# agwi-lab/renderformer

Hardware: AMD Instinct MI355X
Metric: rendered frames/sec at 512×512, renderformer-v1.1-swin-large, 1/2/4/8 MI355X (higher is better)
Workload: dtype fp16+bf16

## Files before the change

### renderformer_amd/csrc/gemm.hip

```cpp
#include <algorithm>
#include <type_traits>
#include <cmath>
#include <math.h>
#include <stdio.h>
#include <stdlib.h>
#include <string.h>

#include "common.h"
#include "env.h"

namespace {

constexpr int BK = 32;
constexpr int P_F16 = 2;

enum Epi { E_BF16 = RF_EPI_BF16, E_F32 = RF_EPI_F32, E_ADD = RF_EPI_ADD_F32, E_SWIGLU = RF_EPI_SWIGLU, E_CONV = 16,
           E_ROPE = 17 };

template <int BM_, int BN_, int WGM_, int WGN_, int STAGES_, int KH_ = 1>
struct Tile {
    static constexpr int BM = BM_, BN = BN_, WGM = WGM_, WGN = WGN_, STAGES = STAGES_, KH = KH_;
    static constexpr int NWAVE = WGM * WGN, THREADS = NWAVE * 64;
    static constexpr int MW = BM / WGM, NWD = BN / WGN, TI = MW / 16, TJ = NWD / 16;
    static constexpr int APIECES = BM / 16;
    static constexpr bool ASHARE = APIECES < NWAVE;
    static constexpr int PA = ASHARE ? 1 : BM / 16 / NWAVE, PB = BN / 16 / NWAVE;
    static constexpr int A_BYTES = BM * BK * 2, B_BYTES = BN * BK * 2;
    static_assert(PA >= 1 && PB >= 1 && (ASHARE || PA * NWAVE * 16 == BM || BM == 288) && PB * NWAVE * 16 == BN,
                  "tile/wave mismatch");
    static_assert(TI >= 1 && TJ >= 2 && TJ % 2 == 0, "wave tile too small");
};

struct EngineArgs {
    const bf16_t* a;
    const bf16_t* a_lo;
    int64_t lda;
    const bf16_t* w;
    const bf16_t* w_lo;
    int64_t ldw;
    int m, n, k;
    int hi, wi, cin_pad, ho, wo, kw, stride, pad;
    uint64_t cin_m, kw_m;
    const bf16_t* zero;
// ... 12 lines not shown
    float elu_alpha;
    float* sk_part;
    int* sk_flag;
    int sk_epoch;
    int group_m;
    const int* gate;
    int halo_lg;
    int* err;
    int spin;
    uint64_t* stamps;
    const uint8_t* sa;
    const uint8_t* sw;
    int ld_sa, ld_sw;
    int persist;
    int l2pf;
    int out_f16;
    int* range;
    bf16_t* xg;
    int64_t ldxg;
    const float* norm_g;
    float* ss_out;
    int xg_f16;
    const float* rs_part;
    float rs_n, rs_eps;
    float* seg_ss;
    int seg_w, seg_n;
    const float* rope_pos;
    int64_t rope_ld;
    int rope_div;
    const float* rope_freqs;
// ... 2 lines not shown
    float rope_qscale;
};

constexpr int PN_SLOTS = RF_PRENORM_SLOTS;


RF_DEV uint32_t pack16(const EngineArgs& p, float lo, float hi) {
    return p.out_f16 ? pack_f16x2(lo, hi) : pack_bf16x2(lo, hi);
}

RF_DEV float unpack16(const EngineArgs& p, uint32_t h) {
    return p.out_f16 ? f16_bits_to_f32((uint16_t)h) : __uint_as_float(h << 16);
}

RF_DEV bool gated_off(const EngineArgs& p) { return p.gate && *p.gate == 0; }

RF_DEV int udiv_m(int x, uint64_t m) { return (int)(((uint64_t)(uint32_t)x * m) >> 32); }
inline uint64_t udiv_magic(int d) { return (1ull << 32) / (uint64_t)d + 1; }


RF_DEV void tile_coords(int tile, int tiles_m, int tiles_n, int group_m, int& tm, int& tn) {
    const int per_group = group_m * tiles_n;
    const int g = tile / per_group, r = tile - g * per_group;
    const int first = g * group_m;
    const int gm = min(tiles_m - first, group_m);
    tm = first + r % gm;
    tn = r / gm;
}

RF_DEV int lds_off(int row, int ch) { return row * 64 + ((ch ^ ((row >> 1) & 3)) << 4); }
// ... 86 lines not shown
    for (int pc = 0; pc < PA; ++pc) {
        int m = m0 + arow[pc];
        const bool ok = m < p.m;
        m = ok ? m : p.m - 1;
        g_img[pc] = g_iy[pc] = g_ix[pc] = 0;
        if constexpr (GATHER) {
            const int ox = m % p.wo, t = m / p.wo;
            g_img[pc] = ok ? t / p.ho : -1;
            g_iy[pc] = (t % p.ho) * p.stride - p.pad;
            g_ix[pc] = ox * p.stride - p.pad;
        }
        a_row[pc] = p.a + (int64_t)m * p.lda;
        a_row_lo[pc] = NTERM == 3 ? p.a_lo + (int64_t)m * p.lda : nullptr;
    }

    auto issue = [&](int kt, int buf) {
#pragma unroll
      for (int h = 0; h < KH; ++h) {
        char* st = smem + buf * STAGE_BYTES + h * HALF_BYTES;
        const int k0 = (kt * KH + h) * BK;
        int cb = k0, ky = 0, kx = 0;
        if constexpr (GATHER) {
            const int tap = udiv_m(k0, p.cin_m);
            cb = k0 - tap * p.cin_pad;
            ky = udiv_m(tap, p.kw_m);
            kx = tap - ky * p.kw;
        }
#pragma unroll
        for (int pc = 0; pc < PA; ++pc) {
            if (!stage_a) break;
            const int piece = wave * PA + pc;
            const int kofs = alc[pc] * 8;
            const bf16_t* sa;
            const bf16_t* sa_lo = nullptr;
            if constexpr (GATHER) {
// ... 587 lines not shown
            case 2: return (j >> 5) * 64 + (j & 31);
            default: return (j >> 5) * 64 + 32 + (j & 31);
        }
    } else {
        switch (r) {
            case 0: return j;
            case 1: return (j >> 5) * 64 + (j & 31);
            default: return (j >> 5) * 64 + 32 + (j & 31);
        }
    }
}
template <int ROWS>
RF_DEV int img(int row, int kh, int ch) { return kh * (ROWS * 64) + row * 64 + ((ch ^ ((row >> 1) & 3)) << 4); }
}

template <int BM, int NTERM, bool GATHER, bool INITC = false>
RF_DEV void phased_mainloop(const EngineArgs& p, char* smem, int m0, int n0, int kbeg, int kend,
                            f32x4 (&acc)[BM / 32][4], bool pre = false) {
    using namespace ph;
    using G = Cfg<BM>;
    constexpr int NREG = G::NREG, NA = G::NA, NX = G::NX, MI = G::MI;
    static_assert(NTERM == 1 || NTERM == P_F16, "phased loop: single-term operands");
    static_assert(!(GATHER && NX), "gathered A: no RAX region");
    constexpr int FA = G::FA, FA1 = G::FA1;
    const int lane = threadIdx.x & 63;
    const int wave = threadIdx.x >> 6;
    const int wr = wave >> 2, wc = wave & 3;
    const int nk = kend - kbeg;
    const bool has_a = BM >= 128 || __builtin_amdgcn_readfirstlane(wave) < BM / 16;
    const bool has_x = NX && (__builtin_amdgcn_readfirstlane(wave) & 3) == 0;

// ... 12 lines not shown
        const int m = m0 + trow[r];
        am[r] = m < p.m ? m : p.m - 1;
        src[r] = p.a + (int64_t)am[r] * p.lda;
        gi[r] = gy[r] = gx[r] = 0;
        if constexpr (GATHER) {
            const int ox = am[r] % p.wo, t = am[r] / p.wo;
            gi[r] = m < p.m ? t / p.ho : -1;
            gy[r] = (t % p.ho) * p.stride - p.pad;
            gx[r] = ox * p.stride - p.pad;
        }
    }
#pragma unroll
    for (int r = NA; r < NREG; ++r) src[r] = p.w + (int64_t)(n0 + trow[r]) * p.ldw;
    const int lch = lane & 3;

    auto issue = [&](int kt, int r) {
        const bool is_a = r < NA || r >= NREG;
        if (is_a && !has_a) return;
        if (r >= NREG && !has_x) return;
        char* base = smem + (kt & 1) * G::TILE + (is_a ? 0 : G::A_IMG);
#pragma unroll
        for (int kh = 0; kh < 2; ++kh) {
            const int row = trow[r];
            const int ch = lch ^ ((row >> 1) & 3);
            const int k0 = (kbeg + kt) * BK2 + kh * 32;
            const bf16_t* g = src[r] + k0 + ch * 8;
            if constexpr (GATHER) {
                if (r < NA) {
                    const int tap = udiv_m(k0, p.cin_m), cb = k0 - tap * p.cin_pad;
                    const int ky = udiv_m(tap, p.kw_m), kx = tap - ky * p.kw;
                    const int iy = gy[r] + ky, ix = gx[r] + kx;
                    const bool ok = gi[r] >= 0 && iy >= 0 && iy < p.hi && ix >= 0 && ix < p.wi;
                    g = ok ? p.a + (((int64_t)gi[r] * p.hi + iy) * p.wi + ix) * p.cin_pad + cb + ch * 8 : p.zero;
                }
            }
            char* dst = base + kh * (is_a ? BM * 64 : 256 * 64) + grow[r] * 64;
            __builtin_amdgcn_global_load_lds(GLB_PTR(void, g), LDS_PTR(void, dst), 16, 0, 0);
        }
    };

// ... 123 lines not shown
                issue(t + 2, 0);
                issue(t + 2, 1);
                if (has_a) wait_vm<4>();
                else wait_vm<2>();
            } else {
                wait_vm<0>();
            }
            sync_in();
            mma(0, 1, fb1);
            sync_out();
        }
    }
    if (!late) __builtin_amdgcn_s_barrier();
}

template <int BM, int NTERM, bool INITC>
RF_DEV void phased3_mainloop(const EngineArgs& p, char* smem, int m0, int n0, int kbeg, int kend,
                             f32x4 (&acc)[BM / 32][4], char* touch_lds = nullptr) {
    using namespace ph;
    using G = Cfg<BM>;
    static_assert(BM <= 128, "three-buffer loop: short tiles");
    constexpr int NREG = 3, FA = G::FA;
    const int lane = threadIdx.x & 63;
    const int wave = threadIdx.x >> 6;
    const int wr = wave >> 2, wc = wave & 3;
    const int nk = kend - kbeg;
    const bool has_a = BM >= 128 || __builtin_amdgcn_readfirstlane(wave) < BM / 16;
    const int jrow = 16 * wave + (lane >> 2);
    int trow[NREG], grow[NREG];
    const bf16_t* src[NREG];
#pragma unroll
    for (int r = 0; r < NREG; ++r) {
        trow[r] = region_row<BM>(r, jrow);
        grow[r] = region_row<BM>(r, 16 * wave);
    }
    {
        const int m = m0 + trow[0];
        src[0] = p.a + (int64_t)(m < p.m ? m : p.m - 1) * p.lda;
    }
#pragma unroll
    for (int r = 1; r < NREG; ++r) src[r] = p.w + (int64_t)(n0 + trow[r]) * p.ldw;
    const int lch = lane & 3;
    auto issue_tile = [&](int kt) {
        char* buf = smem + (kt % 3) * G::TILE;
#pragma unroll
        for (int r = 0; r < NREG; ++r) {
            const bool is_a = r == 0;
            if (is_a && !has_a) continue;
            char* base = buf + (is_a ? 0 : G::A_IMG);
#pragma unroll
            for (int kh = 0; kh < 2; ++kh) {
                const int row = trow[r];
                const int ch = lch ^ ((row >> 1) & 3);
                const int k0 = (kbeg + kt) * BK2 + kh * 32;
                char* dst = base + kh * (is_a ? BM * 64 : 256 * 64) + grow[r] * 64;
                __builtin_amdgcn_global_load_lds(GLB_PTR(void, src[r] + k0 + ch * 8), LDS_PTR(void, dst), 16, 0, 0);
            }
        }
    };
    const int l2pf = touch_lds ? p.l2pf : 0;
    const bf16_t* tsrc;
    {
        const int t = threadIdx.x;
        tsrc = t < BM ? p.a + (int64_t)min(m0 + t, p.m - 1) * p.lda
                      : p.w + (int64_t)(n0 + (t - BM) % 256) * p.ldw;
    }
    auto touch = [&](int kt) {
        const int kk = min(kt + l2pf, nk - 1);
        __builtin_amdgcn_global_load_lds(GLB_PTR(void, tsrc + (kbeg + kk) * BK2), LDS_PTR(void, touch_lds), 4, 0, 0);
    };
    if (INITC && kbeg == 0) {
        load_c_acc<BM / 32, 4>(p, m0 + wr * (BM / 2), n0 + wc * 64, acc);
    } else {
#pragma unroll
        for (int i = 0; i < BM / 32; ++i)
#pragma unroll
            for (int j = 0; j < 4; ++j) acc[i][j] = f32x4{0.f, 0.f, 0.f, 0.f};
    }
    const int frow = lane & 15, fch = lane >> 4;
    bf16x8 fa[FA][2], fb0[2][2], fb1[2][2];
    auto read_a = [&](const char* buf) {
#pragma unroll
        for (int i = 0; i < FA; ++i)
#pragma unroll
            for (int s = 0; s < 2; ++s)
                fa[i][s] = *reinterpret_cast<const bf16x8*>(buf + img<BM>(wr * (BM / 2) + i * 16 + frow, s, fch));
    };
    auto read_b = [&](const char* buf, int ni, bf16x8 (&fb)[2][2]) {
#pragma unroll
        for (int j = 0; j < 2; ++j)
#pragma unroll
            for (int s = 0; s < 2; ++s)
                fb[j][s] = *reinterpret_cast<const bf16x8*>(buf + G::A_IMG + img<256>(wc * 64 + ni * 32 + j * 16 + frow, s, fch));
    };
    auto mma = [&](int ni, const bf16x8 (&fb)[2][2]) {
        __builtin_amdgcn_s_setprio(1);
#pragma unroll
        for (int s = 0; s < 2; ++s)
#pragma unroll
            for (int i = 0; i < FA; ++i)
#pragma unroll
                for (int j = 0; j < 2; ++j) {
                    f32x4& c = acc[i][ni * 2 + j];
                    if constexpr (NTERM == P_F16)
                        c = __builtin_amdgcn_mfma_f32_16x16x32_f16(__builtin_bit_cast(f16x8, fb[j][s]),
                                                                   __builtin_bit_cast(f16x8, fa[i][s]), c, 0, 0, 0);
                    else
                        c = __builtin_amdgcn_mfma_f32_16x16x32_bf16(fb[j][s], fa[i][s], c, 0, 0, 0);
// ... 49 lines not shown
                else wait_vm<6>();
            } else {
                if (has_a) wait_vm<6>();
                else wait_vm<4>();
            }
        } else {
            wait_vm<0>();
        }
        sync_in();
        mma(1, fb1);
        sync_out();
    }
    if (!late) __builtin_amdgcn_s_barrier();
}

template <int BM, int EPI, int NTERM = 1>
__global__ __launch_bounds__(512, 1) void phased3_kernel(EngineArgs p) {
    using TE = Tile<BM, 256, 2, 4, 4>;
#ifdef RF_STUDY
    __shared__ __attribute__((aligned(16))) char smem[3 * ph::Cfg<BM>::TILE + PN_AREA<TE, EPI> + 256];
#else
    __shared__ __attribute__((aligned(16))) char smem[3 * ph::Cfg<BM>::TILE + PN_AREA<TE, EPI>];
#endif
    if (gated_off(p)) return;
    const int tiles_m = (p.m + BM - 1) / BM;
    const int nwg = gridDim.x;
    const int hw = blockIdx.x;
    const int xcd = hw & 7, q = nwg >> 3, r = nwg & 7;
    const int wg = (xcd < r ? xcd * (q + 1) : r * (q + 1) + (xcd - r) * q) + (hw >> 3);
    int tm, tn;
    tile_coords(wg, tiles_m, p.n / ph::BN, p.group_m, tm, tn);
    f32x4 acc[BM / 32][4];
    char* const area = smem + 3 * ph::Cfg<BM>::TILE;
    pn_issue<TE, EPI>(p, area, tm * BM, tn * ph::BN);
#ifdef RF_STUDY
    char* const touch = area + PN_AREA<TE, EPI>;
#else
    char* const touch = nullptr;
#endif
    phased3_mainloop<BM, NTERM, EPI == E_ADD>(p, smem, tm * BM, tn * ph::BN, 0, p.k / ph::BK2, acc, touch);
    engine_epilogue<TE, EPI>(p, tm * BM, tn * ph::BN, acc, area);
}

template <int BM, int EPI, int NTERM, bool GATHER>
__global__ __launch_bounds__(512, 1) void phased_kernel(EngineArgs p) {
    using TE = Tile<BM, 256, 2, 4, 4>;
    static_assert(ph::Cfg<BM>::LDS + PN_AREA<TE, EPI> <= 160 * 1024, "phased tile: over the CU's 160 KiB of LDS");
    __shared__ __attribute__((aligned(16))) char smem[ph::Cfg<BM>::LDS + PN_AREA<TE, EPI>];
    if (gated_off(p)) return;
    const int tiles_m = (p.m + BM - 1) / BM;
    const int nwg = gridDim.x;
    const int hw = blockIdx.x;
    const int xcd = hw & 7, q = nwg >> 3, r = nwg & 7;
    const int wg = (xcd < r ? xcd * (q + 1) : r * (q + 1) + (xcd - r) * q) + (hw >> 3);
    int tm, tn;
    tile_coords(wg, tiles_m, p.n / ph::BN, p.group_m, tm, tn);
    f32x4 acc[BM / 32][4];
    char* const area = smem + ph::Cfg<BM>::LDS;
    pn_issue<TE, EPI>(p, area, tm * BM, tn * ph::BN);
    phased_mainloop<BM, NTERM, GATHER, EPI == E_ADD>(p, smem, tm * BM, tn * ph::BN, 0, p.k / ph::BK2, acc);
    engine_epilogue<TE, EPI>(p, tm * BM, tn * ph::BN, acc, area);
}

RF_DEV void phased_issue01(const EngineArgs& p, char* smem, int m0, int n0, int nk) {
    using namespace ph;
    using G = Cfg<256>;
    const int lane = threadIdx.x & 63, wave = threadIdx.x >> 6;
    const int jrow = 16 * wave + (lane >> 2), lch = lane & 3;
#pragma unroll
    for (int kt = 0; kt < 2; ++kt) {
        if (kt == 1 && nk < 2) break;
#pragma unroll
        for (int r = 0; r < G::NREG; ++r) {
            const bool is_a = r < G::NA;
            const int trow = region_row<256>(r, jrow), grow = region_row<256>(r, 16 * wave);
            const bf16_t* src;
            if (is_a) {
                const int m = m0 + trow;
                src = p.a + (int64_t)(m < p.m ? m : p.m - 1) * p.lda;
            } else {
                src = p.w + (int64_t)(n0 + trow) * p.ldw;
            }
            char* base = smem + (kt & 1) * G::TILE + (is_a ? 0 : G::A_IMG);
#pragma unroll
            for (int kh = 0; kh < 2; ++kh) {
                const int ch = lch ^ ((trow >> 1) & 3);
                const bf16_t* g = src + kt * BK2 + kh * 32 + ch * 8;
                char* dst = base + kh * (256 * 64) + grow * 64;
                __builtin_amdgcn_global_load_lds(GLB_PTR(void, g), LDS_PTR(void, dst), 16, 0, 0);
            }
        }
    }
}

template <int EPI, int NTERM>
__global__ __launch_bounds__(512, 1) void phased_sk_kernel(EngineArgs p) {
    constexpr int TI = 8, TJ = 4, BM = 256, TS = BM * ph::BN;
    using TE = Tile<256, 256, 2, 4, 4>;
    __shared__ __attribute__((aligned(16))) char smem[ph::Cfg<BM>::LDS + PN_AREA<TE, EPI>];
    char* const area = smem + ph::Cfg<BM>::LDS;
    const bool pn = p.xg || p.rs_part;
    if (gated_off(p)) return;
// ... 35 lines not shown
        return;
    }
    uint64_t st[16];
    int ns = 0;
    const bool stamp = p.stamps != nullptr;
    if (stamp) st[ns++] = __builtin_amdgcn_s_memtime();
    while (it < it_end) {
        const int tile = (int)(it / iters), kf = (int)(it % iters);
        const int kl = (int)min((int64_t)iters, kf + (it_end - it));
        int tm, tn;
        tile_coords(tile, tiles_m, tiles_n, p.group_m, tm, tn);
        const int m0 = tm * BM, n0 = tn * ph::BN;
        wait_vm<0>();
        __syncthreads();
        if (pn && kf == 0) pn_issue<TE, EPI>(p, area, m0, n0);
        phased_mainloop<BM, NTERM, false, EPI == E_ADD>(p, smem, m0, n0, kf, kl, acc);
        if (stamp && ns < 14) st[ns++] = __builtin_amdgcn_s_memtime();
        if (kf != 0) {
            const __amdgpu_buffer_rsrc_t rs =
                __builtin_amdgcn_make_buffer_rsrc(p.sk_part + (int64_t)L * TS, 0, TS * 4, 0x00020000);
#pragma unroll
            for (int i = 0; i < TI; ++i)
#pragma unroll
                for (int j = 0; j < TJ; ++j) {
                    const int off = (((wave * TI + i) * TJ + j) * 64 + lane) * 16;
                    __builtin_amdgcn_raw_buffer_store_b128(__builtin_bit_cast(u32x4, acc[i][j]), rs, off, 0, 16);
                }
            asm volatile("s_waitcnt vmcnt(0)" ::: "memory");
            __syncthreads();
            if (threadIdx.x == 0) __hip_atomic_store(p.sk_flag + L, p.sk_epoch, __ATOMIC_RELAXED, __HIP_MEMORY_SCOPE_AGENT);
        } else {
// ... 1323 lines not shown
using T64x256k2 = Tile<64, 256, 2, 4, 3, 2>;
using T64x256w4k2 = Tile<64, 256, 1, 4, 3, 2>;
using T64c = Tile<64, 64, 2, 2, 8>;
using T64x128c = Tile<64, 128, 2, 2, 6>;

int pick_group_m(int tiles_m, int tiles_n, int bm, int bn, int64_t per_xcd, int64_t a_bytes = 0) {
    if (rf::env_set("RF_GEMM_GROUP_M")) return std::max(1, std::min(tiles_m, rf::env_int("RF_GEMM_GROUP_M", 0)));
    if (RF_ENV_ONCE("RF_GEMM_STREAM_RASTER", 1) != 0 && a_bytes > (192ll << 20) && tiles_n <= 8) return std::max(1, std::min(tiles_m, 32 / tiles_n));
    const double g = std::sqrt((double)per_xcd * bn / bm);
    int gm = (int)(g + 0.5);
    gm = std::max(1, std::min(gm, tiles_m));
    if ((int64_t)gm * tiles_n < per_xcd / 2) gm = std::min<int64_t>(tiles_m, (per_xcd + tiles_n - 1) / tiles_n);
    return gm;
}

template <class C, int EPI, int NTERM, bool GATHER = false>
int launch(EngineArgs a, void* stream, const char* what) {
    const int tiles_m = (a.m + C::BM - 1) / C::BM, tiles_n = a.n / C::BN;
    const int nwg = tiles_n * tiles_m;
    a.group_m = pick_group_m(tiles_m, tiles_n, C::BM, C::BN, (nwg + 7) / 8, GATHER ? 0 : (int64_t)a.m * a.k * 2);
    RF_LAUNCH((engine_kernel<C, EPI, NTERM, GATHER, false>), dim3(nwg), dim3(C::THREADS), 0, (hipStream_t)stream,
                       a);
    return rf::check_launch(what);
}

template <class C>
bool halo_ok(EngineArgs& a) {
    if (a.kw != 3 || a.k != 9 * a.cin_pad || a.stride != 1 || a.pad != 1 || a.ho != a.hi || a.wo != a.wi) return false;
    if (a.cin_pad % BK || a.m % C::BM || (a.ho * a.wo) % C::BM) return false;
    const int tw = std::min(C::BM, a.wo);
    if (tw < 16 || (tw & (tw - 1)) || a.wo % tw || C::BM % tw) return false;
    const int th = C::BM / tw;
    if (a.ho % th || (th + 2) * (tw + 2) > Halo<C>::ROWS) return false;
    a.halo_lg = __builtin_ctz(tw);
    return true;
// ... 13 lines not shown
    if constexpr (GATHER && NTERM == P_F16) {
        const bool want = rf::env_int("RF_CONV_HALO", C::BM == 128 && C::NWAVE == 4) != 0;
        if (want && halo_ok<C>(a)) return launch_halo<C, E_CONV>(a, stream, what);
    }
    return launch<C, E_CONV, NTERM, GATHER>(a, stream, what);
}

constexpr int SK_MAX_GRID = 768;
constexpr int64_t SK_PART_FLOATS = (int64_t)256 * 256 * 256;
constexpr int64_t SK_WS_BYTES = SK_PART_FLOATS * 4 + SK_MAX_GRID * 4;

template <class C, int EPI, int NTERM = 1, bool GATHER = false>
int launch_sk(EngineArgs a, int grid, void* stream, const char* what) {
    const int tiles_m = (a.m + C::BM - 1) / C::BM, tiles_n = a.n / C::BN;
    a.group_m = pick_group_m(tiles_m, tiles_n, C::BM, C::BN, ((int64_t)tiles_m * tiles_n + 7) / 8);
    RF_LAUNCH((engine_kernel<C, EPI, NTERM, GATHER, true>), dim3(grid), dim3(C::THREADS), 0,
                       (hipStream_t)stream, a);
    return rf::check_launch(what);
}

int sk_setup(EngineArgs& p, void* workspace, void* stream) {
    p.sk_part = (float*)workspace;
    p.sk_flag = (int*)(p.sk_part + SK_PART_FLOATS);
    p.sk_epoch = rf::next_epoch(p.sk_flag, SK_MAX_GRID * sizeof(int), (hipStream_t)stream);
    if (p.sk_epoch == 0) return RF_ERR_LAUNCH;
    p.err = rf::device_error_word();
    p.spin = rf::spin_limit();
    p.stamps = RF_ENV_ONCE("RF_GEMM_STAMPS", 0) != 0 ? (uint64_t*)(p.sk_part + SK_PART_FLOATS - 65536) : nullptr;
    return RF_OK;
}
// ... 41 lines not shown
enum TileCode : int {
    TC_R128 = 128,
    TC_P256 = 256,
    TC_P288 = 288,
    TC_R64 = 642,
    TC_P64 = 643,
    TC_R64w4 = 644,
    TC_P3_64 = 645,
    TC_R64s6 = 646,
    TC_R96 = 962,
    TC_P96 = 963,
    TC_P3_96 = 964,
    TC_R96s5 = 965,
    TC_R96s6 = 966,
    TC_P128 = 1282,
    TC_P3_128 = 1283,
    TC_R128s4 = 1284,
    TC_R128s5 = 1285,
    TC_R128s6 = 1286,
    TC_R128w8s6 = 1288,
    TC_R256x128 = 2561,
    TC_R64k2 = 6423,
    TC_R64w4k2 = 6443,
    TC_R96k2 = 9623,
    TC_R128k2s3 = 12823,
    TC_R128k2s4 = 12824,
    TC_R128w8k2 = 12884,
};

int pick_cfg(int m, int n, int k, int epilogue = RF_EPI_BF16) {
    if (rf::env_set("RF_GEMM_TILE")) return rf::env_int("RF_GEMM_TILE", 0);
    const bool phased = n % 256 == 0 && k % 64 == 0 && rf::env_int("RF_GEMM_PHASED", 1) != 0;
    const double kk = k / 1024.0;
    const bool add = epilogue == RF_EPI_ADD_F32;
    auto cost = [&](int bm, int bn, int slots, double fixed, double per_k, double add_cost) {
        const int64_t tiles = (int64_t)((m + bm - 1) / bm) * (n / bn);
        const int64_t rounds = (tiles + 256 * slots - 1) / (256 * slots);
        return rounds * (fixed + per_k * kk + (add ? add_cost : 0.0));
    };
    int best = TC_R128;
    const int64_t t128 = (int64_t)((m + 127) / 128) * (n / 128);
    double best_c = t128 <= 256 ? cost(128, 128, 1, 5.5, 13.1, 5.0) : cost(128, 128, 2, 11.0, 14.0, 5.0);
    auto consider = [&](int cfg, double c) {
        if (c < best_c) {
            best_c = c;
            best = cfg;
        }
    };
    if (k % 64 == 0) consider(TC_R128w8k2, cost(128, 128, 1, 6.8, 10.9, 5.0));
    if (n % 256 == 0) consider(TC_R96, cost(96, 256, 1, 2.2, 16.5, 13.0));
    if (phased) {
        consider(TC_P256, cost(256, 256, 1, 11.0, 20.4, 5.0));
        consider(TC_P288, cost(288, 256, 1, 22.5, 22.1, 5.0));
        consider(TC_P128, cost(128, 256, 1, 2.3, 18.4, 5.0));
        consider(TC_P3_96, cost(96, 256, 1, 6.0, 14.4, 5.0));
        consider(TC_P3_64, cost(64, 256, 1, 6.5, 11.8, 5.0));
    }
    return best;
}

__device__ __attribute__((aligned(16))) bf16_t g_zero_row[64];

namespace mx {
constexpr int BM = 256, BN = 256, KS = 128;
constexpr int A_DATA = BM * KS, B_DATA = BN * KS;
constexpr int STAGE = A_DATA + B_DATA + (BM + BN) * 4;
constexpr int TI = 8, TJ = 4;
typedef __attribute__((ext_vector_type(8))) int i32x8;
RF_DEV int off(int row, int ch) { return row * KS + ((ch ^ (row & 7)) << 4); }
}

template <bool INITC>
// ... 298 lines not shown
}

bool persist_on() {
    return RF_ENV_ONCE("RF_GEMM_PERSIST", 1) != 0;
}

bool persist_ragged() {
    return RF_ENV_ONCE("RF_GEMM_PERSIST_RAGGED", 0) != 0;
}

template <int EPI, int NTERM, bool GATHER, int BM = 256>
int launch_phased(EngineArgs a, void* stream, const char* what) {
    const int tiles_m = (a.m + BM - 1) / BM, tiles_n = a.n / 256;
    const int nwg = tiles_n * tiles_m;
    a.group_m = pick_group_m(tiles_m, tiles_n, BM, 256, (nwg + 7) / 8, GATHER ? 0 : (int64_t)a.m * a.k * 2);
    if constexpr (BM == 256 && (NTERM == 1 || NTERM == P_F16) && !GATHER) {
        if (nwg > 256 && persist_on() && (nwg % 256 == 0 || persist_ragged())) {
            a.persist = 1;
            RF_LAUNCH((phased_sk_kernel<EPI, NTERM>), dim3(256), dim3(512), 0, (hipStream_t)stream, a);
            return rf::check_launch(what);
        }
    }
    RF_LAUNCH((phased_kernel<BM, EPI, NTERM, GATHER>), dim3(nwg), dim3(512), 0, (hipStream_t)stream, a);
    return rf::check_launch(what);
}

#ifdef RF_STUDY
int l2pf_dist() {
    return std::max(0, std::min(8, rf::env_int("RF_GEMM_L2PF", 0)));
}
#endif

template <int EPI, int BM, int NT = 1>
int launch_phased3(EngineArgs a, void* stream, const char* what) {
#ifdef RF_STUDY
    a.l2pf = l2pf_dist();
#endif
    const int tiles_m = (a.m + BM - 1) / BM, tiles_n = a.n / 256;
    const int nwg = tiles_n * tiles_m;
    a.group_m = pick_group_m(tiles_m, tiles_n, BM, 256, (nwg + 7) / 8, (int64_t)a.m * a.k * 2);
    RF_LAUNCH((phased3_kernel<BM, EPI, NT>), dim3(nwg), dim3(512), 0, (hipStream_t)stream, a);
    return rf::check_launch(what);
}

template <int EPI, int NT = 1>
int launch_phased_sk(EngineArgs a, int grid, void* stream, const char* what) {
    const int tiles_m = (a.m + 255) / 256, tiles_n = a.n / 256;
    a.group_m = pick_group_m(tiles_m, tiles_n, 256, 256, ((int64_t)tiles_m * tiles_n + 7) / 8);
    RF_LAUNCH((phased_sk_kernel<EPI, NT>), dim3(grid), dim3(512), 0, (hipStream_t)stream, a);
    return rf::check_launch(what);
}

bool use_phased(int n, int k) {
    return rf::env_int("RF_GEMM_PHASED", 1) != 0 && n % 256 == 0 && k % 64 == 0;
}

template <class C>
struct Ring {};
template <int BM>
struct Phased {};
template <int BM>
struct Phased3 {};

enum Pre { PRE_NONE = 0, PRE_N256 = 1, PRE_K64 = 2, PRE_PHASED = 4 };

bool pre_ok(int pre, const EngineArgs& p) {
    return (!(pre & PRE_N256) || p.n % 256 == 0) && (!(pre & PRE_K64) || p.k % 64 == 0) &&
           (!(pre & PRE_PHASED) || use_phased(p.n, p.k));
}

template <int CODE, class LOOP, int PRE, bool F16>
struct Row {};
template <class... R>
struct Rows {};

using TileTable = Rows<
    Row<TC_P256,        Phased<256>,                      PRE_PHASED,          true>,
    Row<TC_P128,        Phased<128>,                      PRE_PHASED,          true>,
    Row<TC_P288,        Phased<288>,                      PRE_PHASED,          true>,
    Row<TC_P256,        Ring<T256>,                       PRE_N256,            false>,
    Row<TC_R128s4,      Ring<Tile<128, 128, 2, 2, 4>>,    PRE_NONE,            false>,
    Row<TC_R128s5,      Ring<Tile<128, 128, 2, 2, 5>>,    PRE_NONE,            false>,
    Row<TC_R256x128,    Ring<T256x128>,                   PRE_NONE,            false>,
    Row<TC_R96,         Ring<T96x256>,                    PRE_N256,            true>,
    Row<TC_R64,         Ring<T64x256>,                    PRE_N256,            false>,
    Row<TC_P3_128,      Phased3<128>,                     PRE_PHASED,          true>,
    Row<TC_P3_96,       Phased3<96>,                      PRE_PHASED,          true>,
    Row<TC_P3_64,       Phased3<64>,                      PRE_PHASED,          true>,
    Row<TC_P96,         Phased<96>,                       PRE_PHASED,          false>,
    Row<TC_P64,         Phased<64>,                       PRE_PHASED,          false>,
    Row<TC_R64w4,       Ring<T64x256w4>,                  PRE_N256,            false>,
    Row<TC_R96s5,       Ring<T96x256s5>,                  PRE_N256,            false>,
    Row<TC_R96s6,       Ring<T96x256s6>,                  PRE_N256,            false>,
    Row<TC_R64s6,       Ring<T64x256s6>,                  PRE_N256,            false>,
    Row<TC_R128s6,      Ring<T128s6>,                     PRE_NONE,            false>,
    Row<TC_R128w8s6,    Ring<T128w8s6>,                   PRE_NONE,            false>,
    Row<TC_R128k2s3,    Ring<T128k2s3>,                   PRE_K64,             false>,
    Row<TC_R128k2s4,    Ring<T128k2s4>,                   PRE_K64,             false>,
    Row<TC_R128w8k2,    Ring<T128w8k2s4>,                 PRE_K64,             true>,
    Row<TC_R96k2,       Ring<T96x256k2>,                  PRE_K64 | PRE_N256,  false>,
    Row<TC_R64k2,       Ring<T64x256k2>,                  PRE_K64 | PRE_N256,  false>,
    Row<TC_R64w4k2,     Ring<T64x256w4k2>,                PRE_K64 | PRE_N256,  false>,
    Row<TC_R128,        Ring<T128>,                       PRE_NONE,            true>>;

template <int NT, class C>
int run_loop(Ring<C>, const EngineArgs& p, int epilogue, void* stream) {
    return with_epi(epilogue, [&](auto e) { return launch<C, decltype(e)::value, NT>(p, stream, "rf_gemm"); });
}
template <int NT, int BM>
int run_loop(Phased<BM>, const EngineArgs& p, int epilogue, void* stream) {
    return with_epi(epilogue, [&](auto e) {
        return launch_phased<decltype(e)::value, NT, false, BM>(p, stream, NT == P_F16 ? "rf_gemm_f16" : "rf_gemm_bf16");
    });
}
template <int NT, int BM>
int run_loop(Phased3<BM>, const EngineArgs& p, int epilogue, void* stream) {
    return with_epi(epilogue, [&](auto e) { return launch_phased3<decltype(e)::value, BM, NT>(p, stream, "rf_gemm"); });
}

template <int NT, int CODE, class LOOP, int PRE, bool F16>
bool try_row(Row<CODE, LOOP, PRE, F16>, int cfg, const EngineArgs& p, int epilogue, void* stream, int& rc) {
    if constexpr (NT == P_F16 && !F16) {
        return false;
    } else {
        if (cfg != CODE || !pre_ok(PRE, p)) return false;
        rc = run_loop<NT>(LOOP{}, p, epilogue, stream);
        return true;
    }
}

template <int NT, class... R>
int run_dp(Rows<R...>, int cfg, const EngineArgs& p, int epilogue, void* stream) {
// ... 88 lines not shown
        out_f16 = 1;
        epilogue = epilogue == RF_EPI_F16 ? RF_EPI_BF16 : RF_EPI_SWIGLU;
    }
    RF_REQUIRE(m > 0 && n > 0 && k > 0, "rf_gemm_bf16: empty problem m=%d n=%d k=%d", m, n, k);
    RF_REQUIRE(k % BK == 0, "rf_gemm_bf16: K=%d must be a multiple of %d", k, BK);
    RF_REQUIRE(n % 128 == 0, "rf_gemm_bf16: N=%d must be a multiple of 128", n);
    RF_REQUIRE(lda % 8 == 0 && ldw % 8 == 0 && lda >= k && ldw >= k, "rf_gemm_bf16: lda/ldw must be >=K and 16-B aligned");
    RF_REQUIRE(((uintptr_t)a & 15) == 0 && ((uintptr_t)w & 15) == 0, "rf_gemm_bf16: operands must be 16-B aligned");
    RF_REQUIRE(epilogue >= RF_EPI_BF16 && epilogue <= RF_EPI_SWIGLU, "rf_gemm_bf16: bad epilogue %d", epilogue);
    RF_REQUIRE(ldc >= (epilogue == RF_EPI_SWIGLU ? n / 2 : n) && ldc % 4 == 0, "rf_gemm_bf16: ldc too small/unaligned");
    RF_REQUIRE(((uintptr_t)c & 7) == 0, "rf_gemm_bf16: output must be 8-B aligned");
    EngineArgs p = norm ? *norm : EngineArgs{};
    dense_args(p, a, lda, w, ldw, m, n, k, c, ldc);
    p.bias = bias;
    p.gate = gate;
    p.out_f16 = out_f16;
    p.range = (out_f16 || (p.xg && p.xg_f16)) ? rf::range_word() : nullptr;
    const char* what = f16 ? "rf_gemm_f16" : "rf_gemm_bf16";
    const bool ws_ok = workspace && ws_bytes >= SK_WS_BYTES;
#ifdef RF_STUDY
    if (const int qm = norm ? 0 : quad_mode(m, n, k, lda, ldw, epilogue)) {
        return f16 ? run_quad<P_F16>(p, epilogue, qm, workspace, ws_bytes, stream, what)
                   : run_quad<1>(p, epilogue, qm, workspace, ws_bytes, stream, what);
    }
#else
    if (rf::env_int("RF_GEMM_QUAD", 0) > 0) return rf::study_only("rf_gemm: RF_GEMM_QUAD");
#endif
    if (ws_ok && skph(m, n, k)) {
        if (const int rc = sk_setup(p, workspace, stream)) return rc;
        const int64_t tiles = (int64_t)((m + 255) / 256) * (n / 256);
// ... 110 lines not shown
    EngineArgs p{};
    dense_args(p, a, lda, w, ldw, m, n, k, c, ldc);
    p.rs_part = ss;
    p.rs_n = (float)norm_dim;
    p.rs_eps = eps;
    p.seg_ss = norm_w ? seg_ss : nullptr;
    p.seg_w = seg_w;
    p.seg_n = n_seg;
    p.rope_pos = pos;
    p.rope_ld = ld_pos;
    p.rope_div = pos ? pos_div : 1;
    p.rope_freqs = freqs;
    p.rope_nf = pos ? n_freqs : 1;
    p.rope_g = norm_w;
    p.rope_qscale = q_scale;
    const bool f16 = operand_dtype == RF_DT_F16;
    const int cfg = pick_cfg(m, n, k, RF_EPI_BF16);
    if (cfg == TC_P288 && use_phased(n, k)) {
        return f16 ? launch_phased<E_ROPE, P_F16, false, 288>(p, stream, "rf_gemm_qk_rope")
                   : launch_phased<E_ROPE, 1, false, 288>(p, stream, "rf_gemm_qk_rope");
    }
    const bool t96 = n % 256 == 0 && cfg != TC_R128w8k2;
    if (t96) return f16 ? launch_rope<T96x256, P_F16>(p, stream) : launch_rope<T96x256, 1>(p, stream);
    return f16 ? launch_rope<T128w8k2s4, P_F16>(p, stream) : launch_rope<T128w8k2s4, 1>(p, stream);
}

extern "C" int rf_gemm_bf16_if(const int* flag, const void* a, int64_t lda, const void* w, int64_t ldw, void* c,
                               int64_t ldc, const float* bias, int m, int n, int k, int epilogue, void* workspace,
                               int64_t ws_bytes, void* stream) {
    RF_REQUIRE(flag, "rf_gemm_bf16_if: null flag");
    return gemm_bf16(a, lda, w, ldw, c, ldc, bias, m, n, k, epilogue, workspace, ws_bytes, stream, flag);
}
// ... 496 lines not shown
```

Baseline: 92.38.

## Add 192x128 three-buffer phased GEMM tile and per-block K-rotation of the main loop

Generalizes the three-buffer phased mainloop to support a 192x128 tile with three 40-KiB K buffers and adds it as a cost-model candidate in tile selection. Separately adds K-loop rotation: each workgroup starts its K iteration at an offset derived from blockIdx, so concurrent blocks read different K slices of the operands. The rotation is meant to spread memory-channel and L2 traffic. It is auto-enabled only for ring 128x128 and phased 128/256 configs with 128-256 tiles and at least 8 K tiles. The new tile raises LDS use and shifts which kernel the cost model picks.

After: 92.51 (median of 6 runs). No clear change (+0.1%).

```diff
diff --git a/renderformer_amd/csrc/gemm.hip b/renderformer_amd/csrc/gemm.hip
--- a/renderformer_amd/csrc/gemm.hip
+++ b/renderformer_amd/csrc/gemm.hip
@@ -26,7 +26,7 @@
     static constexpr bool ASHARE = APIECES < NWAVE;
     static constexpr int PA = ASHARE ? 1 : BM / 16 / NWAVE, PB = BN / 16 / NWAVE;
     static constexpr int A_BYTES = BM * BK * 2, B_BYTES = BN * BK * 2;
-    static_assert(PA >= 1 && PB >= 1 && (ASHARE || PA * NWAVE * 16 == BM || BM == 288) && PB * NWAVE * 16 == BN,
+    static_assert(PA >= 1 && PB >= 1 && (ASHARE || PA * NWAVE * 16 == BM || BM == 288 || BM == 192) && PB * NWAVE * 16 == BN,
                   "tile/wave mismatch");
     static_assert(TI >= 1 && TJ >= 2 && TJ % 2 == 0, "wave tile too small");
 };
@@ -69,6 +69,8 @@
     int ld_sa, ld_sw;
     int persist;
     int l2pf;
+    int krot;
+    int krot_req;
     int out_f16;
     int* range;
     bf16_t* xg;
@@ -101,6 +103,15 @@
 }
 
 RF_DEV bool gated_off(const EngineArgs& p) { return p.gate && *p.gate == 0; }
+
+RF_DEV int krot_first(const EngineArgs& p, int kbeg, int kend, int iters) {
+    return (p.krot && kbeg == 0 && kend == iters) ? (int)((blockIdx.x & 7u) * (unsigned)iters) >> 3 : 0;
+}
+RF_DEV int krot_tile(int kt, int first, int iters) {
+    const int g = kt + first;
+    return g >= iters ? g - iters : g;
+}
+RF_DEV int krot_k0(int kt, int wrap, int bk, int k) { return kt * bk - (kt >= wrap ? k : 0); }
 
 RF_DEV int udiv_m(int x, uint64_t m) { return (int)(((uint64_t)(uint32_t)x * m) >> 32); }
 inline uint64_t udiv_magic(int d) { return (1ull << 32) / (uint64_t)d + 1; }
@@ -217,11 +228,13 @@
         a_row_lo[pc] = NTERM == 3 ? p.a_lo + (int64_t)m * p.lda : nullptr;
     }
 
+    const int kiters = p.k / (BK * KH);
+    const int kfirst = GATHER ? 0 : krot_first(p, kbeg, kend, kiters);
     auto issue = [&](int kt, int buf) {
 #pragma unroll
       for (int h = 0; h < KH; ++h) {
         char* st = smem + buf * STAGE_BYTES + h * HALF_BYTES;
-        const int k0 = (kt * KH + h) * BK;
+        const int k0 = ((GATHER ? kt : krot_tile(kt, kfirst, kiters)) * KH + h) * BK;
         int cb = k0, ky = 0, kx = 0;
         if constexpr (GATHER) {
             const int tap = udiv_m(k0, p.cin_m);
@@ -839,7 +852,7 @@
 RF_DEV int img(int row, int kh, int ch) { return kh * (ROWS * 64) + row * 64 + ((ch ^ ((row >> 1) & 3)) << 4); }
 }
 
-template <int BM, int NTERM, bool GATHER, bool INITC = false>
+template <int BM, int NTERM, bool GATHER, bool INITC = false, bool ROT = true>
 RF_DEV void phased_mainloop(const EngineArgs& p, char* smem, int m0, int n0, int kbeg, int kend,
                             f32x4 (&acc)[BM / 32][4], bool pre = false) {
     using namespace ph;
@@ -882,6 +895,13 @@
     for (int r = NA; r < NREG; ++r) src[r] = p.w + (int64_t)(n0 + trow[r]) * p.ldw;
     const int lch = lane & 3;
 
+    constexpr bool KROT = ROT && !GATHER;
+    const int kfirst = KROT ? krot_first(p, kbeg, kend, p.k / BK2) : 0;
+    const int kwrap = p.k / BK2 - kfirst;
+    if constexpr (KROT) {
+#pragma unroll
+        for (int r = 0; r < NREG + NX; ++r) src[r] += kfirst * BK2;
+    }
     auto issue = [&](int kt, int r) {
         const bool is_a = r < NA || r >= NREG;
         if (is_a && !has_a) return;
@@ -891,7 +911,7 @@
         for (int kh = 0; kh < 2; ++kh) {
             const int row = trow[r];
             const int ch = lch ^ ((row >> 1) & 3);
-            const int k0 = (kbeg + kt) * BK2 + kh * 32;
+            const int k0 = (KROT ? krot_k0(kbeg + kt, kwrap, BK2, p.k) : (kbeg + kt) * BK2) + kh * 32;
             const bf16_t* g = src[r] + k0 + ch * 8;
             if constexpr (GATHER) {
                 if (r < NA) {
@@ -1045,46 +1065,71 @@
     if (!late) __builtin_amdgcn_s_barrier();
 }
 
-template <int BM, int NTERM, bool INITC>
+namespace ph {
+template <int BM, int BN>
+struct Cfg3 {
+    static_assert((BN == 256 && BM <= 128) || (BN == 128 && BM == 192), "three-buffer loop: short tiles, or 192x128");
+    static constexpr int WGN = BN / 64, WGM = 8 / WGN;
+    static constexpr int MW = BM / WGM, FA = MW / 16;
+    static constexpr int A_IMG = BM * 128;
+    static constexpr int TILE = A_IMG + BN * 128;
+    static constexpr int LDS = 3 * TILE;
+    static constexpr int OPT_REG = BN == 256 ? 0 : 1, OPT_A = BN == 256 ? BM / 16 : (BM - 128) / 16;
+    static constexpr int NA = BN == 256 ? 1 : 2;
+};
+template <int BM, int BN>
+RF_DEV int region_row3(int r, int j) {
+    if constexpr (BN == 256) return region_row<BM>(r, j);
+    else return r == 1 ? 128 + (j & 63) : j;
+}
+}
+static_assert(ph::Cfg3<192, 128>::LDS == 120 * 1024, "192x128 tile: three 40-KiB K-tile buffers");
+
+template <int BM, int NTERM, bool INITC, int BN = 256>
 RF_DEV void phased3_mainloop(const EngineArgs& p, char* smem, int m0, int n0, int kbeg, int kend,
-                             f32x4 (&acc)[BM / 32][4], char* touch_lds = nullptr) {
+                             f32x4 (&acc)[ph::Cfg3<BM, BN>::FA][4], char* touch_lds = nullptr) {
     using namespace ph;
-    using G = Cfg<BM>;
-    static_assert(BM <= 128, "three-buffer loop: short tiles");
-    constexpr int NREG = 3, FA = G::FA;
+    using G = Cfg3<BM, BN>;
+    constexpr int NREG = 3, FA = G::FA, NA = G::NA;
     const int lane = threadIdx.x & 63;
     const int wave = threadIdx.x >> 6;
-    const int wr = wave >> 2, wc = wave & 3;
+    const int wr = wave / G::WGN, wc = wave % G::WGN;
     const int nk = kend - kbeg;
-    const bool has_a = BM >= 128 || __builtin_amdgcn_readfirstlane(wave) < BM / 16;
+    const bool has_a = G::OPT_A >= 8 || __builtin_amdgcn_readfirstlane(wave) < G::OPT_A;
     const int jrow = 16 * wave + (lane >> 2);
     int trow[NREG], grow[NREG];
     const bf16_t* src[NREG];
 #pragma unroll
     for (int r = 0; r < NREG; ++r) {
-        trow[r] = region_row<BM>(r, jrow);
-        grow[r] = region_row<BM>(r, 16 * wave);
-    }
-    {
-        const int m = m0 + trow[0];
-        src[0] = p.a + (int64_t)(m < p.m ? m : p.m - 1) * p.lda;
-    }
-#pragma unroll
-    for (int r = 1; r < NREG; ++r) src[r] = p.w + (int64_t)(n0 + trow[r]) * p.ldw;
+        trow[r] = region_row3<BM, BN>(r, jrow);
+        grow[r] = region_row3<BM, BN>(r, 16 * wave);
+    }
+#pragma unroll
+    for (int r = 0; r < NA; ++r) {
+        const int m = m0 + trow[r];
+        src[r] = p.a + (int64_t)(m < p.m ? m : p.m - 1) * p.lda;
+    }
+#pragma unroll
+    for (int r = NA; r < NREG; ++r) src[r] = p.w + (int64_t)(n0 + trow[r]) * p.ldw;
     const int lch = lane & 3;
+    const int kfirst = krot_first(p, kbeg, kend, p.k / BK2);
+    const int kwrap = p.k / BK2 - kfirst;
+#pragma unroll
+    for (int r = 0; r < NREG; ++r) src[r] += kfirst * BK2;
     auto issue_tile = [&](int kt) {
         char* buf = smem + (kt % 3) * G::TILE;
+        const int kg0 = krot_k0(kbeg + kt, kwrap, BK2, p.k);
 #pragma unroll
         for (int r = 0; r < NREG; ++r) {
-            const bool is_a = r == 0;
-            if (is_a && !has_a) continue;
+            const bool is_a = r < NA;
+            if (r == G::OPT_REG && !has_a) continue;
             char* base = buf + (is_a ? 0 : G::A_IMG);
 #pragma unroll
             for (int kh = 0; kh < 2; ++kh) {
                 const int row = trow[r];
                 const int ch = lch ^ ((row >> 1) & 3);
-                const int k0 = (kbeg + kt) * BK2 + kh * 32;
-                char* dst = base + kh * (is_a ? BM * 64 : 256 * 64) + grow[r] * 64;
+                const int k0 = kg0 + kh * 32;
+                char* dst = base + kh * (is_a ? BM * 64 : BN * 64) + grow[r] * 64;
                 __builtin_amdgcn_global_load_lds(GLB_PTR(void, src[r] + k0 + ch * 8), LDS_PTR(void, dst), 16, 0, 0);
             }
         }
@@ -1094,17 +1139,18 @@
     {
         const int t = threadIdx.x;
         tsrc = t < BM ? p.a + (int64_t)min(m0 + t, p.m - 1) * p.lda
-                      : p.w + (int64_t)(n0 + (t - BM) % 256) * p.ldw;
+                      : p.w + (int64_t)(n0 + (t - BM) % BN) * p.ldw;
     }
     auto touch = [&](int kt) {
         const int kk = min(kt + l2pf, nk - 1);
-        __builtin_amdgcn_global_load_lds(GLB_PTR(void, tsrc + (kbeg + kk) * BK2), LDS_PTR(void, touch_lds), 4, 0, 0);
+        __builtin_amdgcn_global_load_lds(GLB_PTR(void, tsrc + krot_tile(kbeg + kk, kfirst, p.k / BK2) * BK2),
+                                         LDS_PTR(void, touch_lds), 4, 0, 0);
     };
     if (INITC && kbeg == 0) {
-        load_c_acc<BM / 32, 4>(p, m0 + wr * (BM / 2), n0 + wc * 64, acc);
+        load_c_acc<FA, 4>(p, m0 + wr * G::MW, n0 + wc * 64, acc);
     } else {
 #pragma unroll
-        for (int i = 0; i < BM / 32; ++i)
+        for (int i = 0; i < FA; ++i)
 #pragma unroll
             for (int j = 0; j < 4; ++j) acc[i][j] = f32x4{0.f, 0.f, 0.f, 0.f};
     }
@@ -1115,14 +1161,14 @@
         for (int i = 0; i < FA; ++i)
 #pragma unroll
             for (int s = 0; s < 2; ++s)
-                fa[i][s] = *reinterpret_cast<const bf16x8*>(buf + img<BM>(wr * (BM / 2) + i * 16 + frow, s, fch));
+                fa[i][s] = *reinterpret_cast<const bf16x8*>(buf + img<BM>(wr * G::MW + i * 16 + frow, s, fch));
     };
     auto read_b = [&](const char* buf, int ni, bf16x8 (&fb)[2][2]) {
 #pragma unroll
         for (int j = 0; j < 2; ++j)
 #pragma unroll
             for (int s = 0; s < 2; ++s)
-                fb[j][s] = *reinterpret_cast<const bf16x8*>(buf + G::A_IMG + img<256>(wc * 64 + ni * 32 + j * 16 + frow, s, fch));
+                fb[j][s] = *reinterpret_cast<const bf16x8*>(buf + G::A_IMG + img<BN>(wc * 64 + ni * 32 + j * 16 + frow, s, fch));
     };
     auto mma = [&](int ni, const bf16x8 (&fb)[2][2]) {
         __builtin_amdgcn_s_setprio(1);
@@ -1202,13 +1248,15 @@
     if (!late) __builtin_amdgcn_s_barrier();
 }
 
-template <int BM, int EPI, int NTERM = 1>
+template <int BM, int EPI, int NTERM = 1, int BN = 256>
 __global__ __launch_bounds__(512, 1) void phased3_kernel(EngineArgs p) {
-    using TE = Tile<BM, 256, 2, 4, 4>;
+    using G3 = ph::Cfg3<BM, BN>;
+    using TE = Tile<BM, BN, G3::WGM, G3::WGN, 4>;
+    static_assert(G3::LDS + PN_AREA<TE, EPI> + 256 <= 160 * 1024, "phased3 tile: over the CU's 160 KiB of LDS");
 #ifdef RF_STUDY
-    __shared__ __attribute__((aligned(16))) char smem[3 * ph::Cfg<BM>::TILE + PN_AREA<TE, EPI> + 256];
+    __shared__ __attribute__((aligned(16))) char smem[G3::LDS + PN_AREA<TE, EPI> + 256];
 #else
-    __shared__ __attribute__((aligned(16))) char smem[3 * ph::Cfg<BM>::TILE + PN_AREA<TE, EPI>];
+    __shared__ __attribute__((aligned(16))) char smem[G3::LDS + PN_AREA<TE, EPI>];
 #endif
     if (gated_off(p)) return;
     const int tiles_m = (p.m + BM - 1) / BM;
@@ -1217,17 +1265,17 @@
     const int xcd = hw & 7, q = nwg >> 3, r = nwg & 7;
     const int wg = (xcd < r ? xcd * (q + 1) : r * (q + 1) + (xcd - r) * q) + (hw >> 3);
     int tm, tn;
-    tile_coords(wg, tiles_m, p.n / ph::BN, p.group_m, tm, tn);
-    f32x4 acc[BM / 32][4];
-    char* const area = smem + 3 * ph::Cfg<BM>::TILE;
-    pn_issue<TE, EPI>(p, area, tm * BM, tn * ph::BN);
+    tile_coords(wg, tiles_m, p.n / BN, p.group_m, tm, tn);
+    f32x4 acc[G3::FA][4];
+    char* const area = smem + G3::LDS;
+    pn_issue<TE, EPI>(p, area, tm * BM, tn * BN);
 #ifdef RF_STUDY
     char* const touch = area + PN_AREA<TE, EPI>;
 #else
     char* const touch = nullptr;
 #endif
-    phased3_mainloop<BM, NTERM, EPI == E_ADD>(p, smem, tm * BM, tn * ph::BN, 0, p.k / ph::BK2, acc, touch);
-    engine_epilogue<TE, EPI>(p, tm * BM, tn * ph::BN, acc, area);
+    phased3_mainloop<BM, NTERM, EPI == E_ADD, BN>(p, smem, tm * BM, tn * BN, 0, p.k / ph::BK2, acc, touch);
+    engine_epilogue<TE, EPI>(p, tm * BM, tn * BN, acc, area);
 }
 
 template <int BM, int EPI, int NTERM, bool GATHER>
@@ -1251,6 +1299,7 @@
 }
 
 RF_DEV void phased_issue01(const EngineArgs& p, char* smem, int m0, int n0, int nk) {
+    const int kfirst = krot_first(p, 0, nk, nk);
     using namespace ph;
     using G = Cfg<256>;
     const int lane = threadIdx.x & 63, wave = threadIdx.x >> 6;
@@ -1273,7 +1322,7 @@
 #pragma unroll
             for (int kh = 0; kh < 2; ++kh) {
                 const int ch = lch ^ ((trow >> 1) & 3);
-                const bf16_t* g = src + kt * BK2 + kh * 32 + ch * 8;
+                const bf16_t* g = src + krot_tile(kt, kfirst, nk) * BK2 + kh * 32 + ch * 8;
                 char* dst = base + kh * (256 * 64) + grow * 64;
                 __builtin_amdgcn_global_load_lds(GLB_PTR(void, g), LDS_PTR(void, dst), 16, 0, 0);
             }
@@ -1339,7 +1388,7 @@
         wait_vm<0>();
         __syncthreads();
         if (pn && kf == 0) pn_issue<TE, EPI>(p, area, m0, n0);
-        phased_mainloop<BM, NTERM, false, EPI == E_ADD>(p, smem, m0, n0, kf, kl, acc);
+        phased_mainloop<BM, NTERM, false, EPI == E_ADD, false>(p, smem, m0, n0, kf, kl, acc);
         if (stamp && ns < 14) st[ns++] = __builtin_amdgcn_s_memtime();
         if (kf != 0) {
             const __amdgpu_buffer_rsrc_t rs =
@@ -2693,11 +2742,21 @@
     return gm;
 }
 
+enum KrotReq { KROT_OFF = 0, KROT_ON = 1, KROT_AUTO = 2 };
+int krot_request() { return rf::env_set("RF_GEMM_KROT") ? (rf::env_int("RF_GEMM_KROT", 0) != 0 ? KROT_ON : KROT_OFF) : KROT_AUTO; }
+int krot_resolve(int req, bool won, int64_t tiles, int k_tiles) {
+    if (req != KROT_AUTO) return req == KROT_ON;
+    return won && tiles >= 128 && tiles <= 256 && k_tiles >= 8;
+}
+template <class C>
+constexpr bool krot_won_ring = C::BM == 128 && C::BN == 128 && C::NWAVE == 8 && C::KH == 2;
+
 template <class C, int EPI, int NTERM, bool GATHER = false>
 int launch(EngineArgs a, void* stream, const char* what) {
     const int tiles_m = (a.m + C::BM - 1) / C::BM, tiles_n = a.n / C::BN;
     const int nwg = tiles_n * tiles_m;
     a.group_m = pick_group_m(tiles_m, tiles_n, C::BM, C::BN, (nwg + 7) / 8, GATHER ? 0 : (int64_t)a.m * a.k * 2);
+    a.krot = GATHER ? 0 : krot_resolve(a.krot_req, krot_won_ring<C>, nwg, a.k / (BK * C::KH));
     RF_LAUNCH((engine_kernel<C, EPI, NTERM, GATHER, false>), dim3(nwg), dim3(C::THREADS), 0, (hipStream_t)stream,
                        a);
     return rf::check_launch(what);
@@ -2741,6 +2800,7 @@
 int launch_sk(EngineArgs a, int grid, void* stream, const char* what) {
     const int tiles_m = (a.m + C::BM - 1) / C::BM, tiles_n = a.n / C::BN;
     a.group_m = pick_group_m(tiles_m, tiles_n, C::BM, C::BN, ((int64_t)tiles_m * tiles_n + 7) / 8);
+    a.krot = GATHER ? 0 : krot_resolve(a.krot_req, false, (int64_t)tiles_m * tiles_n, a.k / (BK * C::KH));
     RF_LAUNCH((engine_kernel<C, EPI, NTERM, GATHER, true>), dim3(grid), dim3(C::THREADS), 0,
                        (hipStream_t)stream, a);
     return rf::check_launch(what);
@@ -2812,6 +2872,7 @@
     TC_R96s5 = 965,
     TC_R96s6 = 966,
     TC_P128 = 1282,
+    TC_P3_192 = 1921,
     TC_P3_128 = 1283,
     TC_R128s4 = 1284,
     TC_R128s5 = 1285,
@@ -2826,7 +2887,7 @@
     TC_R128w8k2 = 12884,
 };
 
-int pick_cfg(int m, int n, int k, int epilogue = RF_EPI_BF16) {
+int pick_cfg(int m, int n, int k, int epilogue = RF_EPI_BF16, bool p3_192 = true) {
     if (rf::env_set("RF_GEMM_TILE")) return rf::env_int("RF_GEMM_TILE", 0);
     const bool phased = n % 256 == 0 && k % 64 == 0 && rf::env_int("RF_GEMM_PHASED", 1) != 0;
     const double kk = k / 1024.0;
@@ -2854,6 +2915,7 @@
         consider(TC_P3_96, cost(96, 256, 1, 6.0, 14.4, 5.0));
         consider(TC_P3_64, cost(64, 256, 1, 6.5, 11.8, 5.0));
     }
+    if (p3_192 && k % 64 == 0 && rf::env_int("RF_GEMM_PHASED", 1) != 0) consider(TC_P3_192, cost(192, 128, 1, 7.7, 12.6, 5.0));
     return best;
 }
 
@@ -3182,6 +3244,7 @@
     const int tiles_m = (a.m + BM - 1) / BM, tiles_n = a.n / 256;
     const int nwg = tiles_n * tiles_m;
     a.group_m = pick_group_m(tiles_m, tiles_n, BM, 256, (nwg + 7) / 8, GATHER ? 0 : (int64_t)a.m * a.k * 2);
+    a.krot = GATHER ? 0 : krot_resolve(a.krot_req, BM == 256 || BM == 128, nwg, a.k / ph::BK2);
     if constexpr (BM == 256 && (NTERM == 1 || NTERM == P_F16) && !GATHER) {
         if (nwg > 256 && persist_on() && (nwg % 256 == 0 || persist_ragged())) {
             a.persist = 1;
@@ -3199,15 +3262,16 @@
 }
 #endif
 
-template <int EPI, int BM, int NT = 1>
+template <int EPI, int BM, int NT = 1, int BN = 256>
 int launch_phased3(EngineArgs a, void* stream, const char* what) {
 #ifdef RF_STUDY
     a.l2pf = l2pf_dist();
 #endif
-    const int tiles_m = (a.m + BM - 1) / BM, tiles_n = a.n / 256;
+    const int tiles_m = (a.m + BM - 1) / BM, tiles_n = a.n / BN;
     const int nwg = tiles_n * tiles_m;
-    a.group_m = pick_group_m(tiles_m, tiles_n, BM, 256, (nwg + 7) / 8, (int64_t)a.m * a.k * 2);
-    RF_LAUNCH((phased3_kernel<BM, EPI, NT>), dim3(nwg), dim3(512), 0, (hipStream_t)stream, a);
+    a.group_m = pick_group_m(tiles_m, tiles_n, BM, BN, (nwg + 7) / 8, (int64_t)a.m * a.k * 2);
+    a.krot = krot_resolve(a.krot_req, false, nwg, a.k / ph::BK2);
+    RF_LAUNCH((phased3_kernel<BM, EPI, NT, BN>), dim3(nwg), dim3(512), 0, (hipStream_t)stream, a);
     return rf::check_launch(what);
 }
 
@@ -3215,6 +3279,7 @@
 int launch_phased_sk(EngineArgs a, int grid, void* stream, const char* what) {
     const int tiles_m = (a.m + 255) / 256, tiles_n = a.n / 256;
     a.group_m = pick_group_m(tiles_m, tiles_n, 256, 256, ((int64_t)tiles_m * tiles_n + 7) / 8);
+    a.krot = krot_resolve(a.krot_req, false, (int64_t)tiles_m * tiles_n, a.k / ph::BK2);
     RF_LAUNCH((phased_sk_kernel<EPI, NT>), dim3(grid), dim3(512), 0, (hipStream_t)stream, a);
     return rf::check_launch(what);
 }
@@ -3227,14 +3292,15 @@
 struct Ring {};
 template <int BM>
 struct Phased {};
-template <int BM>
+template <int BM, int BN = 256>
 struct Phased3 {};
 
-enum Pre { PRE_NONE = 0, PRE_N256 = 1, PRE_K64 = 2, PRE_PHASED = 4 };
+enum Pre { PRE_NONE = 0, PRE_N256 = 1, PRE_K64 = 2, PRE_PHASED = 4, PRE_PHASED_ON = 8 };
 
 bool pre_ok(int pre, const EngineArgs& p) {
     return (!(pre & PRE_N256) || p.n % 256 == 0) && (!(pre & PRE_K64) || p.k % 64 == 0) &&
-           (!(pre & PRE_PHASED) || use_phased(p.n, p.k));
+           (!(pre & PRE_PHASED) || use_phased(p.n, p.k)) &&
+           (!(pre & PRE_PHASED_ON) || rf::env_int("RF_GEMM_PHASED", 1) != 0);
 }
 
 template <int CODE, class LOOP, int PRE, bool F16>
@@ -3255,6 +3321,7 @@
     Row<TC_P3_128,      Phased3<128>,                     PRE_PHASED,          true>,
     Row<TC_P3_96,       Phased3<96>,                      PRE_PHASED,          true>,
     Row<TC_P3_64,       Phased3<64>,                      PRE_PHASED,          true>,
+    Row<TC_P3_192,      Phased3<192, 128>,                PRE_K64 | PRE_PHASED_ON, true>,
     Row<TC_P96,         Phased<96>,                       PRE_PHASED,          false>,
     Row<TC_P64,         Phased<64>,                       PRE_PHASED,          false>,
     Row<TC_R64w4,       Ring<T64x256w4>,                  PRE_N256,            false>,
@@ -3281,9 +3348,9 @@
         return launch_phased<decltype(e)::value, NT, false, BM>(p, stream, NT == P_F16 ? "rf_gemm_f16" : "rf_gemm_bf16");
     });
 }
-template <int NT, int BM>
-int run_loop(Phased3<BM>, const EngineArgs& p, int epilogue, void* stream) {
-    return with_epi(epilogue, [&](auto e) { return launch_phased3<decltype(e)::value, BM, NT>(p, stream, "rf_gemm"); });
+template <int NT, int BM, int BN>
+int run_loop(Phased3<BM, BN>, const EngineArgs& p, int epilogue, void* stream) {
+    return with_epi(epilogue, [&](auto e) { return launch_phased3<decltype(e)::value, BM, NT, BN>(p, stream, "rf_gemm"); });
 }
 
 template <int NT, int CODE, class LOOP, int PRE, bool F16>
@@ -3402,6 +3469,7 @@
     dense_args(p, a, lda, w, ldw, m, n, k, c, ldc);
     p.bias = bias;
     p.gate = gate;
+    p.krot_req = krot_request();
     p.out_f16 = out_f16;
     p.range = (out_f16 || (p.xg && p.xg_f16)) ? rf::range_word() : nullptr;
     const char* what = f16 ? "rf_gemm_f16" : "rf_gemm_bf16";
@@ -3542,8 +3610,9 @@
     p.rope_nf = pos ? n_freqs : 1;
     p.rope_g = norm_w;
     p.rope_qscale = q_scale;
+    p.krot_req = krot_request();
     const bool f16 = operand_dtype == RF_DT_F16;
-    const int cfg = pick_cfg(m, n, k, RF_EPI_BF16);
+    const int cfg = pick_cfg(m, n, k, RF_EPI_BF16, false);
     if (cfg == TC_P288 && use_phased(n, k)) {
         return f16 ? launch_phased<E_ROPE, P_F16, false, 288>(p, stream, "rf_gemm_qk_rope")
                    : launch_phased<E_ROPE, 1, false, 288>(p, stream, "rf_gemm_qk_rope");
```
